# ComputationalPhysiology/oasisx

Measured on AMD Instinct MI355X. Metric: time-steps/sec, 3D Taylor-Green 128^3 P2-P1 (with pressure-CG SpMV GB/s in roofline), higher is better.
Workload: dtype f64

## Files before the change

include/oasisx_hip.h:

```cpp
#ifndef OASISX_HIP_H
#define OASISX_HIP_H

#include <stddef.h>
#include <stdint.h>

#ifdef __cplusplus
extern "C" {
#endif

#define OX_KV 2
#define OX_ROW_BLOCK_WAVES 8
#define OX_ROW_BLOCK_LDS (134 * 1024)
#define OX_SLICE 64

#define OX_CONVERGED_RTOL 2
#define OX_CONVERGED_ATOL 3
#define OX_CONVERGED_ITS 4
#define OX_DIVERGED_ITS (-3)
#define OX_DIVERGED_DTOL (-4)
#define OX_DIVERGED_BREAKDOWN (-5)
#define OX_DIVERGED_NANORINF (-9)

#define OX_KSP_CG 1
#define OX_KSP_BCGS 2
// ... 12 lines not shown
  const int32_t *cols;
  double *vals;
  const uint16_t *cols16;
  const int32_t *cbase;
  const uint8_t *vcode;
  const double *vdict;
  const int32_t *ib_slices;
  int32_t n_interior;
  int32_t n_wb_interior;
  const int64_t *ps_ptr;
  const uint32_t *ps_code;
  const int32_t *ps_base;
  const int32_t *wb_slices;
  const uint16_t *wb_waves;
  const int64_t *wb_ptr;
  const int32_t *wlist;
  const int64_t *wt_ptr;
  const uint16_t *wcode;
  const uint8_t *wvcode;
  int32_t n_wblocks;
  int32_t w_max;
  int32_t levels;
  int32_t w_cap;
} ox_sell;
#define OX_SPMV_LEVELS(mask) (32 | ((mask) & 31))

typedef struct {
  int32_t gdim;
  int32_t reserved;
  int64_t n_cells;
  const double *geom;
} ox_cells;

typedef struct {
  int32_t n_slices;
  int32_t nd;
  const int64_t *adj_ptr;
  const int32_t *adj_cell;
  const uint8_t *adj_loc;
} ox_adj;

typedef struct ox_dist ox_dist;
typedef struct ox_mg ox_mg;

typedef struct {
  int32_t reason[4];
  int32_t its[4];
  double rnorm[4];
// ... 90 lines not shown
int ox_value_dictionary(const double *vals, int64_t n_slots, int ncomp, void *codes, double *dict, int *n_dict,
                        void *stream);
int ox_pair_stream_size(const ox_sell *A, const int32_t *row_len, int64_t *ps_ptr, int64_t *n_codes, void *stream);
int ox_window_retile(const ox_sell *A, const int64_t *wt_ptr, const void *src, int elem_bytes, void *dst, void *stream);
int ox_pair_stream_fill(const ox_sell *A, const int32_t *row_len, int64_t *ps_ptr, uint32_t *ps_code,
                        int32_t *ps_base, int64_t *n_wide, void *stream);
int ox_gather_images(const double *src, int64_t n_src, const int32_t *image_dof, int64_t n_images, int ncomp, double *dst,
                     void *stream);
int ox_malloc(size_t bytes, void **out);
int ox_free(void *p);
int ox_memset(void *p, int value, size_t bytes, void *stream);
int ox_synchronize(void *stream);

int ox_version(void);
const char *ox_last_error(void);
int ox_sell_kv(void);
int ox_device_info(int *n_cu, char *name, int name_len);

int ox_spmv(const ox_sell *A, const double *x, double *y, int ncomp, const ox_dist *dist,
            void *stream);

int ox_sell_compress_cols(const ox_sell *A, uint16_t *cols16, int32_t *cbase, int64_t *n_compressed,
                          void *stream);

int ox_spmv_multi(int v2s, int gdim, const ox_sell *A, const double *x, const double *base, double scale,
                  double *y, const ox_dist *dist, void *stream);
int ox_assemble_rect(int family, int row_degree, int col_degree, const ox_cells *cells, const ox_adj *adj,
                     const uint8_t *adj_pos, int pw, const ox_sell *A, void *stream);

int ox_axpby(int64_t n, double a, const double *x, double b, const double *y, double *z,
             void *stream);
int ox_dot(int64_t n_rows, int ncomp, const double *x, const double *y, double *out_host,
           const ox_dist *dist, void *stream);

int ox_set_bc(double *b, const int32_t *dofs, const double *g, int64_t n, int ncomp, int comp,
              void *stream);

int ox_scatter_add(double *b, const int32_t *rows, const double *y, int64_t n, int ncomp, int comp,
                   double scale, void *stream);

int ox_zero_rows(const ox_sell *A, const int32_t *rows, int64_t n, double diag, void *stream);
int ox_zero_rows_au(const ox_sell *A, const int32_t *rows, int64_t n, double diag, double *au,
                    const double *u1, int ncomp, void *stream);
int ox_zero_rows_cols(const ox_sell *A, const uint8_t *is_bc, double diag, void *stream);

int ox_assemble_matrix(int kind, const ox_cells *cells, const ox_space_info *space, const ox_sell *A, int row_blocks,
// ... 228 lines not shown
```

oasisx_amd/_lib.py:

```python
from __future__ import annotations

import ctypes as C
import os

_HERE = os.path.dirname(os.path.abspath(__file__))
LIB_PATH = os.environ.get("OX_LIB_PATH") or os.path.join(_HERE, "liboasisx_hip.so")

KSP_CG, KSP_BCGS, KSP_CG_SINGLE, KSP_BCGS_MERGED, KSP_CG_MERGED = 1, 2, 3, 4, 5
KSP_CG_MG = 6
MG_MAX_DEGREE = 8
ROW_BLOCK_WAVES, ROW_BLOCK_LDS = 8, 134 * 1024
CONVERGED_RTOL, CONVERGED_ATOL, CONVERGED_ITS = 2, 3, 4
DIVERGED_ITS, DIVERGED_DTOL, DIVERGED_BREAKDOWN, DIVERGED_NANORINF = -3, -4, -5, -9


class OasisxHipError(RuntimeError):
    pass


class ox_sell(C.Structure):
    _fields_ = [
        ("n_rows", C.c_int64),
        ("n_cols", C.c_int64),
        ("n_slices", C.c_int32),
# ... 2 lines not shown
        ("cols", C.c_void_p),
        ("vals", C.c_void_p),
        ("cols16", C.c_void_p),
        ("cbase", C.c_void_p),
        ("vcode", C.c_void_p),
        ("vdict", C.c_void_p),
        ("ib_slices", C.c_void_p),
        ("n_interior", C.c_int32),
        ("n_wb_interior", C.c_int32),
        ("ps_ptr", C.c_void_p),
        ("ps_code", C.c_void_p),
        ("ps_base", C.c_void_p),
        ("wb_slices", C.c_void_p),
        ("wb_waves", C.c_void_p),
        ("wb_ptr", C.c_void_p),
        ("wlist", C.c_void_p),
        ("wt_ptr", C.c_void_p),
        ("wcode", C.c_void_p),
        ("wvcode", C.c_void_p),
        ("n_wblocks", C.c_int32),
        ("w_max", C.c_int32),
        ("levels", C.c_int32),
        ("w_cap", C.c_int32),
    ]


class ox_window_info(C.Structure):
    _fields_ = [
        ("n_wblocks", C.c_int32),
        ("w_max", C.c_int32),
        ("n_list", C.c_int64),
        ("n_tiles", C.c_int64),
        ("n_over_16bit", C.c_int64),
        ("wb_slices", C.c_void_p),
        ("wb_waves", C.c_void_p),
        ("wb_ptr", C.c_void_p),
        ("wlist", C.c_void_p),
        ("wt_ptr", C.c_void_p),
        ("wcode", C.c_void_p),
    ]


class ox_cells(C.Structure):
    _fields_ = [
        ("gdim", C.c_int32),
        ("reserved", C.c_int32),
# ... 207 lines not shown
    "ox_mesh_create_periodic": (_I, [_P, _L, _P, _P, _L, _L, _I, _I, _I, C.POINTER(_D), C.POINTER(_P)]),
    "ox_mesh_destroy": (_I, [_P]),
    "ox_space_create": (_I, [_P, _I, _I, C.POINTER(_P)]),
    "ox_space_create_ordered": (_I, [_P, _I, _I, _I, C.POINTER(_P)]),
    "ox_mesh_create_sub": (_I, [_P, _L, _P, _L, _I, _I, C.POINTER(_D), C.POINTER(_D), _I, _I, _L, C.POINTER(_P)]),
    "ox_space_create_part": (_I, [_P, _I, _I, _P, _L, _I, _L, C.POINTER(_P)]),
    "ox_space_view": (_I, [_P, C.POINTER(ox_space_info)]),
    "ox_space_windows": (_I, [_P, C.POINTER(ox_window_info)]),
    "ox_space_windows_split": (_I, [_P, _I, C.POINTER(ox_window_info)]),
    "ox_space_destroy": (_I, [_P]),
    "ox_rect_create": (_I, [_P, _P, C.POINTER(_P)]),
    "ox_rect_view": (_I, [_P, C.POINTER(ox_rect_info)]),
    "ox_rect_destroy": (_I, [_P]),
    "ox_value_dictionary": (_I, [_P, _L, _I, _P, _P, C.POINTER(_I), _P]),
    "ox_pair_stream_size": (_I, [C.POINTER(ox_sell), _P, _P, C.POINTER(_L), _P]),
    "ox_pair_stream_fill": (_I, [C.POINTER(ox_sell), _P, _P, _P, _P, C.POINTER(_L), _P]),
    "ox_gather_images": (_I, [_P, _L, _P, _L, _I, _P, _P]),
    "ox_malloc": (_I, [C.c_size_t, C.POINTER(_P)]),
    "ox_free": (_I, [_P]),
    "ox_memset": (_I, [_P, _I, C.c_size_t, _P]),
    "ox_synchronize": (_I, [_P]),
    "ox_spmv": (_I, [C.POINTER(ox_sell), _P, _P, _I, _P, _P]),
    "ox_sell_compress_cols": (_I, [C.POINTER(ox_sell), _P, _P, C.POINTER(_L), _P]),
    "ox_spmv_multi": (_I, [_I, _I, C.POINTER(ox_sell), _P, _P, _D, _P, _P, _P]),
    "ox_assemble_rect": (_I, [_I, _I, _I, C.POINTER(ox_cells), C.POINTER(ox_adj), _P, _I, C.POINTER(ox_sell), _P]),
    "ox_axpby": (_I, [_L, _D, _P, _D, _P, _P, _P]),
    "ox_dot": (_I, [_L, _I, _P, _P, C.POINTER(_D), _P, _P]),
    "ox_set_bc": (_I, [_P, _P, _P, _L, _I, _I, _P]),
    "ox_scatter_add": (_I, [_P, _P, _P, _L, _I, _I, _D, _P]),
    "ox_zero_rows": (_I, [C.POINTER(ox_sell), _P, _L, _D, _P]),
    "ox_zero_rows_au": (_I, [C.POINTER(ox_sell), _P, _L, _D, _P, _P, _I, _P]),
    "ox_zero_rows_cols": (_I, [C.POINTER(ox_sell), _P, _D, _P]),
    "ox_assemble_matrix": (_I, [_I, C.POINTER(ox_cells), C.POINTER(ox_space_info), C.POINTER(ox_sell), _I, _P]),
    "ox_assemble_weights": (_I, [_I, C.POINTER(ox_cells), C.POINTER(ox_adj), _L, _P, _P]),
    "ox_assemble_load_vector": (_I, [C.POINTER(ox_cells), C.POINTER(ox_adj), _L, _I, _I, _P, _P, _P, _P]),
    "ox_assemble_first": (_I, [C.POINTER(ox_cells), C.POINTER(ox_space_info), C.POINTER(ox_sell), C.POINTER(ox_sell),
                               C.POINTER(ox_sell), C.POINTER(ox_first_args), _I, _P]),
    "ox_eddy_viscosity": (_I, [_I, _I, C.POINTER(ox_cells), _P, _P, _D, _P, _P]),
    "ox_eddy_viscosity_damped": (_I, [_I, _I, C.POINTER(ox_cells), _P, _P, _D, C.POINTER(ox_vandriest), _P, _P]),
    "ox_viscosity_law": (_I, [_I, _I, C.POINTER(ox_cells), _P, _P, C.POINTER(_D), _I, _P, _P]),
    "ox_assemble_stress_transpose": (_I, [_I, C.POINTER(ox_cells), _P, C.POINTER(ox_adj), _L, _P, _P, _D, _P, _P]),
    "ox_flow_cells": (_I, [_I, C.POINTER(ox_cells), _P, _P, _P, _D, _D, _P, _P, _P, _P]),
    "ox_flow_reduce": (_I, [_L, _P, _P, _L, _L, _P]),
    "ox_stats_accumulate": (_I, [_I, _L, _P, _L, _D, _D, _P, _P, _P]),
    "ox_profile_cells": (_I, [_I, C.POINTER(ox_cells), _P, _I, _I, C.POINTER(_P), C.POINTER(_L), _P, _P, _L, _P, _P, _P]),
    "ox_profile_update": (_I, [_I, _L, _P, _P, _P, _D, _D, _I, _P, _P, _P, _P, _P]),
# ... 117 lines not shown
```

oasisx_amd/csrc/ox_ksp.hip:

```cpp
#include "ox_kernels.h"
#include "ox_ksp_dev.h"
#include "ox_p2p.h"
#include <type_traits>

struct KspPart2 {
  const double *partial;
  int nparts, nv;
};

__device__ __forceinline__ void ksp_gather2(const double *__restrict__ partial, int nparts, int nv, const KspPart2 &B,
                                            double (&v)[OX_MAX_NV]) {
  ox_gather_partials(partial, nparts, nv, v);
  if (B.nv > 0) {
    double w[OX_MAX_NV];
    ox_gather_partials(B.partial, B.nparts, B.nv, w);
#pragma unroll
    for (int i = 0; i < OX_MAX_NV; ++i)
#pragma unroll
      for (int j = 0; j < OX_MAX_NV; ++j)
        if (j == i - nv && j < B.nv) v[i] = w[j];
  }
}


// ... 1569 lines not shown
  } else {
    V.r = vec[0], V.rhat = vec[1], V.p = vec[2], V.v = vec[3], V.s = vec[4], V.t = vec[5];
    if (guess && !ax0) {
      if (ox_spmv_dist(A, x, V.t, NC, OX_EPI_NONE, nullptr, nullptr, nullptr, nullptr, dist, st)) return -1;
    }
    hipLaunchKernelGGL((k_bcgs_init<NC>), dim3(C.nb), dim3(256), 0, st, n, b, x, (guess && ax0) ? ax0 : V.t, C.dinv, V.r,
                       V.rhat, V.p, V.v, guess, C.partial);
    OX_LAUNCH_CHECK();
    KSP_SYNC(PH_BCGS_INIT, C.partial, C.nb, 2 * NC);
  }
  bool first = true;
  int it = 0;
  bool tail_done = false;
  for (;;) {
    tail_done = false;
    if (ksp_iterate<NC>(C, V, P, check_every, ahead && NC == 1, it, first, H)) return -1;
    int live = -1;
    if (NC > 1 && !hs->done) live = ksp_last_live(hs, NC);
    if (live >= 0) {
      double *const *cv = C.narrow;
      KspVecs W{};
      double *src[8] = {V.x, V.r, V.z, V.p, V.q, V.rhat, V.v, nullptr};
      double **dst[8] = {&W.x, &W.r, &W.z, &W.p, &W.q, &W.rhat, &W.v, nullptr};
      if (cg) src[2] = nullptr;
      if (cgs) {
        src[2] = V.u, dst[2] = &W.u;
        src[4] = V.s, dst[4] = &W.s;
        src[5] = V.w, dst[5] = &W.w;
        src[6] = nullptr;
      }
      for (int i = 0; i < 7; ++i) {
        *dst[i] = cv[i];
        if (!src[i]) continue;
        hipLaunchKernelGGL(k_extract_col, dim3(C.nb), dim3(256), 0, st, n, src[i], NC, live, cv[i]);
        OX_LAUNCH_CHECK();
      }
      if (!cgs) {
        W.s = cv[2];
        W.t = cv[4];
      }
      KspParams P1 = P;
      P1.nc = 1;
      P1.c0 = live;
      it += check_every;
      if (ksp_iterate<1>(C, W, P1, check_every, ahead, it, first, H)) return -1;
      if (cg) {
        hipLaunchKernelGGL((k_cg_update2<1>), dim3(C.nb), dim3(256), 0, st, n, C.S, P1.c0, W.x, W.r, C.D, W.p, 1);
// ... 93 lines not shown
```

oasisx_amd/csrc/ox_spmv.hip:

```cpp
#include "ox_common.h"
#include "ox_kernels.h"
#include <stdlib.h>
#include <type_traits>

thread_local char ox_err_buf[512] = "";

extern "C" int ox_version(void) { return 101; }
extern "C" const char *ox_last_error(void) { return ox_err_buf; }
extern "C" int ox_sell_kv(void) { return OX_KV; }

extern "C" int ox_device_info(int *n_cu, char *name, int name_len) {
  int dev = 0;
  OX_HIP(hipGetDevice(&dev));
  hipDeviceProp_t p;
  OX_HIP(hipGetDeviceProperties(&p, dev));
  if (n_cu) *n_cu = p.multiProcessorCount;
  if (name && name_len > 0) {
    strncpy(name, p.gcnArchName, name_len - 1);
    name[name_len - 1] = 0;
  }
  return 0;
}

template <int NC, int EPI, int VAR>
// ... 44 lines not shown
      if (VAR & 4) {
        const unsigned cc = __builtin_nontemporal_load(vcp + (size_t)k * 64);
        v.x = dict[cc & 0xff];
        v.y = dict[cc >> 8];
      } else if (VAR & 1) {
        const v2d vv = __builtin_nontemporal_load(reinterpret_cast<const v2d *>(vp + (size_t)k * 64));
        v.x = vv.x;
        v.y = vv.y;
      } else {
        v = vp[(size_t)k * 64];
      }
      return v;
    };
    auto mac = [&](double2 v, int c0, int c1) {
      const double *x0 = x + (size_t)c0 * NC;
      const double *x1 = x + (size_t)c1 * NC;
#pragma unroll
      for (int cc = 0; cc < NC; ++cc) acc[cc] = fma(v.x, x0[cc], acc[cc]);
#pragma unroll
      for (int cc = 0; cc < NC; ++cc) acc[cc] = fma(v.y, x1[cc], acc[cc]);
    };
    const int2 *__restrict__ cb =
        (VAR & 2) ? reinterpret_cast<const int2 *>(A.cbase) + (base >> 7) : nullptr;
    if ((VAR & 2) && cb[0].x >= 0) {
      const v2h *__restrict__ hp = reinterpret_cast<const v2h *>(A.cols16 + base) + lane;
#pragma unroll 4
      for (int k = 0; k < npair; ++k) {
        const double2 v = load_vals(k);
        const v2h d = __builtin_nontemporal_load(hp + (size_t)k * 64);
        const int2 b = cb[k];
        const int dx = d.x, dy = d.y;
        mac(v, ((dx & 0x8000) ? b.y : b.x) + (dx & 0x7fff), ((dy & 0x8000) ? b.y : b.x) + (dy & 0x7fff));
      }
    } else {
      const int2 *__restrict__ cp = reinterpret_cast<const int2 *>(A.cols + base) + lane;
#pragma unroll 4
      for (int k = 0; k < npair; ++k) {
        const double2 v = load_vals(k);
        int2 c;
        if (VAR & 1) {
          const v2i ci = __builtin_nontemporal_load(reinterpret_cast<const v2i *>(cp + (size_t)k * 64));
          c.x = ci.x;
          c.y = ci.y;
        } else {
          c = cp[(size_t)k * 64];
        }
        mac(v, c.x, c.y);
// ... 393 lines not shown
    if (threadIdx.x == 0) {
#pragma unroll
      for (int i = 0; i < NV; ++i) partial[(size_t)blockIdx.x * NV + i] = s[i];
    }
  }
}

#include <mutex>
static const int *ox_zero_flag(hipStream_t st) {
  static std::mutex mu;
  static int *z[16] = {};
  int dev = 0;
  if (hipGetDevice(&dev) != hipSuccess || dev < 0 || dev >= 16) return nullptr;
  std::lock_guard<std::mutex> lock(mu);
  if (!z[dev]) {
    int *p = nullptr;
    if (hipMalloc(&p, 64) != hipSuccess) return nullptr;
    if (hipMemsetAsync(p, 0, 64, st) != hipSuccess || hipStreamSynchronize(st) != hipSuccess) return nullptr;
    z[dev] = p;
  }
  return z[dev];
}

#define OX_SPMV_DEFAULT_VARIANT 31
static inline int spmv_levels(const ox_sell *A) { return (A->levels & 32) ? (A->levels & 31) : OX_SPMV_DEFAULT_VARIANT; }

static int spmv_window_cap(const ox_sell *A, int ncomp, const int32_t *list) {
  if (list && !(A->ib_slices && (list == A->ib_slices || list == A->ib_slices + A->n_interior))) return 0;
  if (!(spmv_levels(A) & 16) || !A->wcode || !A->wt_ptr || !A->wlist || !A->wb_ptr || !A->wb_slices ||
      !A->wb_waves || A->n_wblocks <= 0 || ncomp < 1 || ncomp > 3)
    return 0;
  const int dflt = ncomp == 1 ? 6144 : (ncomp == 2 ? 3072 : 2176);
  const int cap = A->w_cap > 0 ? A->w_cap : dflt;
  return A->w_max < cap ? A->w_max : cap;
}
static inline int spmv_window_grid_n(int nblocks) { return (nblocks + 7) & ~7; }
static inline void spmv_window_range(const ox_sell *A, const int32_t *list, int n_list, int *first, int *count) {
  if (!list) *first = 0, *count = A->n_wblocks;
  else if (list == A->ib_slices && n_list == A->n_interior) *first = 0, *count = A->n_wb_interior;
  else *first = A->n_wb_interior, *count = A->n_wblocks - A->n_wb_interior;
}

static thread_local OxEpiDinv g_epi_dinv{nullptr, nullptr};
void ox_spmv_set_epilogue_dinv(const uint8_t *code, const double *dict) { g_epi_dinv = OxEpiDinv{code, dict}; }

static int spmv_launch_list(const ox_sell *A, const double *x, double *y, int ncomp, int epi,
                            const double *dinv, const double *aux, double *partial, const int *done,
                            hipStream_t st, const int32_t *list, int n_list) {
  const int nblk = list ? ox_spmv_blocks_n(n_list) : ox_spmv_blocks(A);
  if (nblk == 0) return 0;
  const int lv = spmv_levels(A);
  int var = (A->cols16 && A->cbase) ? (lv & 7) : (lv & 1);
  const bool pairs = (lv & 8) && A->ps_ptr && A->ps_code && A->ps_base;
  if ((var & 6) != 6 || !A->vcode || !A->vdict || A->n_dict < 1 || A->n_dict > 256) var &= 3;
  else var = 7;
  const int w_cap = pairs ? 0 : spmv_window_cap(A, ncomp, list);
  if (w_cap > 0) {
    const bool codes = var == 7 && A->wvcode;
    int wb0 = 0, wbn = 0;
    spmv_window_range(A, list, n_list, &wb0, &wbn);
    if (wbn == 0) return 0;
    const int wgrid = spmv_window_grid_n(wbn);
    const size_t lds = (size_t)w_cap * ncomp * sizeof(double);
#define OX_WIN_CASE(NC, E)                                                                                          \
  if (ncomp == NC && epi == E) {                                                                                    \
    auto go = [&](auto kern) -> int {                                                                               \
      if (lds > 48 * 1024)                                                                                          \
        OX_HIP(hipFuncSetAttribute(reinterpret_cast<const void *>(kern), hipFuncAttributeMaxDynamicSharedMemorySize, \
                                   (int)lds));                                                                      \
      if (ox_prof_on) ox_prof_start(OX_TAG_SPMV(NC, E), st, A->n_rows);                                             \
      hipLaunchKernelGGL(kern, dim3(wgrid), dim3(256), lds, st, *A, x, y, dinv, aux, partial, done, w_cap, g_epi_dinv, wb0, wbn); \
      if (ox_prof_on) ox_prof_stop(st);                                                                             \
      OX_LAUNCH_CHECK();                                                                                            \
      return 0;                                                                                                     \
    };                                                                                                              \
    return codes ? go(k_spmv_win<NC, E, 5>) : go(k_spmv_win<NC, E, 1>);                                             \
  }
#define OX_WIN_NC(NC)                                                                                   \
  OX_WIN_CASE(NC, OX_EPI_NONE) OX_WIN_CASE(NC, OX_EPI_DOT) OX_WIN_CASE(NC, OX_EPI_BCGS_V) OX_WIN_CASE(NC, OX_EPI_BCGS_T) \
  OX_WIN_CASE(NC, OX_EPI_BCGS_T5) OX_WIN_CASE(NC, OX_EPI_CG_M2)
    OX_WIN_NC(1) OX_WIN_NC(2) OX_WIN_NC(3)
#undef OX_WIN_NC
#undef OX_WIN_CASE
  }
#define OX_SPMV_LAUNCH(NC, E, V)                                                                   \
  hipLaunchKernelGGL((k_spmv<NC, E, V>), dim3(nblk), dim3(256), 0, st, *A, x, y, dinv, aux, partial, done, list, n_list, g_epi_dinv)
#define OX_SPMV_CASE(NC, E)                                                                     \
  if (ncomp == NC && epi == E) {                                                                \
    if (ox_prof_on) ox_prof_start(OX_TAG_SPMV(NC, E), st, A->n_rows);                                      \
    if (var == 7 && pairs) {                                                                    \
      const int *dz = done ? done : ox_zero_flag(st);                                             \
      if (!dz) OX_FAIL("ox_spmv: no device flag");                                              \
      hipLaunchKernelGGL((k_spmv_ps<NC, E>), dim3(nblk), dim3(256), 0, st, *A, x, y, dinv, aux, partial, dz, list, n_list, g_epi_dinv); \
    } else if (var == 7) OX_SPMV_LAUNCH(NC, E, 7);                                              \
    else if (var == 3) OX_SPMV_LAUNCH(NC, E, 3);                                                \
    else if (var == 2) OX_SPMV_LAUNCH(NC, E, 2);                                                \
    else if (var == 1) OX_SPMV_LAUNCH(NC, E, 1);                                                \
    else OX_SPMV_LAUNCH(NC, E, 0);                                                              \
    if (ox_prof_on) ox_prof_stop(st);                                                           \
    OX_LAUNCH_CHECK();                                                                          \
    return 0;                                                                                   \
  }
#define OX_SPMV_NC(NC)               \
  OX_SPMV_CASE(NC, OX_EPI_NONE)      \
  OX_SPMV_CASE(NC, OX_EPI_DOT)       \
  OX_SPMV_CASE(NC, OX_EPI_BCGS_V)    \
  OX_SPMV_CASE(NC, OX_EPI_BCGS_T)    \
  OX_SPMV_CASE(NC, OX_EPI_BCGS_T5)   \
  OX_SPMV_CASE(NC, OX_EPI_CG_M2)
  OX_SPMV_NC(1) OX_SPMV_NC(2) OX_SPMV_NC(3)
#undef OX_SPMV_NC
#undef OX_SPMV_CASE
  OX_FAIL("ox_spmv: unsupported ncomp=%d epi=%d", ncomp, epi);
}

int ox_spmv_launch(const ox_sell *A, const double *x, double *y, int ncomp, int epi,
                   const double *dinv, const double *aux, double *partial, const int *done,
                   hipStream_t st) {
  return spmv_launch_list(A, x, y, ncomp, epi, dinv, aux, partial, done, st, nullptr, 0);
}

static bool ox_overlap_on(const ox_sell *A, const ox_dist *dist) {
  if (!(dist && dist->n_peers > 0 && A->ib_slices && A->n_interior > 0)) return false;
  if (dist->overlap >= 0) return dist->overlap != 0;
  return !(dist->comm && !dist->p2p && !dist->halo_cb);
}

static int spmv_parts_of(const ox_sell *A, int ncomp, const int32_t *list, int n_list) {
  const bool pairs = (spmv_levels(A) & 8) && A->ps_ptr && A->ps_code && A->ps_base;
  if (!pairs && spmv_window_cap(A, ncomp, list) > 0) {
    int wb0 = 0, wbn = 0;
    spmv_window_range(A, list, n_list, &wb0, &wbn);
    return wbn == 0 ? 0 : spmv_window_grid_n(wbn);
  }
  return list ? ox_spmv_blocks_n(n_list) : ox_spmv_blocks(A);
// ... 76 lines not shown
extern "C" int ox_sell_compress_cols(const ox_sell *A, uint16_t *cols16, int32_t *cbase,
                                     int64_t *n_compressed, void *stream) {
  if (!A || !cols16 || !cbase) OX_FAIL("ox_sell_compress_cols: null argument");
  hipStream_t st = ox_stream(stream);
  if (n_compressed) *n_compressed = 0;
  if (A->n_slices == 0) return 0;
  unsigned long long *cnt = nullptr;
  if (n_compressed) {
    OX_HIP(hipMalloc(&cnt, sizeof(*cnt)));
    OX_HIP(hipMemsetAsync(cnt, 0, sizeof(*cnt), st));
  }
  hipLaunchKernelGGL(k_compress_cols, dim3((A->n_slices + 3) / 4), dim3(256), 0, st, *A, cols16, cbase, cnt);
  OX_LAUNCH_CHECK();
  if (n_compressed) {
    unsigned long long h = 0;
    OX_HIP(hipMemcpyAsync(&h, cnt, sizeof(h), hipMemcpyDeviceToHost, st));
    OX_HIP(hipStreamSynchronize(st));
    OX_HIP(hipFree(cnt));
    *n_compressed = (int64_t)h;
  }
  return 0;
}

template <int GD, int V2S, bool DICT>
__global__ __launch_bounds__(256) void k_spmv_multi(ox_sell A, const double *__restrict__ x,
                                                    const double *__restrict__ base, double scale,
                                                    double *__restrict__ y) {
  __shared__ double dict[DICT ? 256 : 1];
  if constexpr (DICT) {
    if ((int)threadIdx.x < A.n_dict) dict[threadIdx.x] = A.vdict[threadIdx.x];
    __syncthreads();
  }
  const int ngroups = (A.n_slices + 3) >> 2;
  const int chunk = (ngroups + 7) >> 3;
  const int g = (blockIdx.x & 7) * chunk + (blockIdx.x >> 3);
  if ((int)(blockIdx.x >> 3) >= chunk || g >= ngroups) return;
  const int slice = __builtin_amdgcn_readfirstlane(g * 4 + (threadIdx.x >> 6)), lane = threadIdx.x & 63;
  if (slice >= A.n_slices) return;
  const int64_t row = (int64_t)slice * 64 + lane;
  const int64_t sbase = A.slice_ptr[slice];
  const int npair = (int)((A.slice_ptr[slice + 1] - sbase) >> 7);
  const int2 *__restrict__ cp = reinterpret_cast<const int2 *>(A.cols + sbase) + lane;
  double acc[GD];
#pragma unroll
  for (int d = 0; d < GD; ++d) acc[d] = 0.0;
  auto mac = [&](const double (&v)[2 * GD], int c0, int c1) {
// ... 513 lines not shown
```

oasisx_amd/fem.py:

```python
from __future__ import annotations

import ctypes as C
import itertools

import numpy as np
import torch

from . import _lib
from .mesh import Mesh

KV = 2
SLICE = 64
default_scalar_type = np.float64


def local_edges(gdim: int):
    return [(1, 2), (0, 2), (0, 1)] if gdim == 2 else [(2, 3), (1, 3), (1, 2), (0, 3), (0, 2), (0, 1)]


import os as _os


def default_tile_bits(mesh: Mesh) -> int:
    env = _os.environ.get("OX_TILE_BITS")
# ... 144 lines not shown
    for k in per.axes:
        cut[k] = float(per.hi[k] - per.atol[k])
    keep = (X < cut).all(dim=2)
    x = torch.full((n, d), float("nan"), dtype=torch.float64, device=dev)
    x[cd0[keep]] = X[keep]
    return x


class SellPattern:

    def __init__(self, n_rows, n_cols, slice_ptr, cols, row_len, widths, nnz=None, row_blk=None):
        self.n_rows, self.n_cols = int(n_rows), int(n_cols)
        self.slice_ptr = slice_ptr
        self.cols = cols
        self.row_len = row_len
        self.widths = widths
        self.n_slices = int(widths.shape[0])
        self.size = int(cols.shape[0])
        self.nnz = int(row_len.sum().item()) if nnz is None else int(nnz)
        self.device = cols.device
        self.dist = None
        self.cols16 = self.cbase = None
        self.frac16 = 0.0
        self.ib_slices, self.n_interior = None, 0
        w = torch.from_numpy(widths.astype(np.int64))
        order = torch.argsort(w, stable=True)
        ws = w[order]
        uw, counts = torch.unique_consecutive(ws, return_counts=True)
        self.bin_width, self.bin_ptr = merge_small_bins(uw.numpy().astype(np.int32),
                                                        np.concatenate([[0], np.cumsum(counts.numpy())]).astype(np.int64))
        self.bin_slices = order.to(torch.int32).to(self.device)
        if row_blk is None:
            bp, big = row_blocks(widths)
            row_blk = (torch.from_numpy(bp).to(self.device), big)
        self.row_blk_ptr, self.row_blk_entries = row_blk
        self.n_row_blocks = int(self.row_blk_ptr.shape[0]) - 1

    def split_interior(self, n_owned: int):
        if self.n_slices == 0 or self.size == 0:
            return
        width = torch.from_numpy(self.widths.astype(np.int64)).to(self.device) * SLICE
        sl = torch.repeat_interleave(torch.arange(self.n_slices, device=self.device), width)
        ghost = torch.zeros(self.n_slices, dtype=torch.int32, device=self.device)
        ghost.index_put_((sl,), (self.cols >= n_owned).to(torch.int32), accumulate=True)
        interior = torch.nonzero(ghost == 0).reshape(-1)
        boundary = torch.nonzero(ghost > 0).reshape(-1)
# ... 94 lines not shown
            bs = torch.repeat_interleave(blk_of_slice[s0:s1], slot_per_slice[s0:s1])
            code = torch.searchsorted(ukey, bs * ncols + self.cols[a:b].to(torch.int64)) - wb_ptr[bs]
            code = torch.where(big[bs], torch.zeros_like(code), code)
            wcode[a:b] = (code & 0xffff).to(torch.int32).to(torch.int16)
        npair = width // KV
        wt_ptr = torch.zeros(ns + 1, dtype=torch.int64, device=dev)
        wt_ptr[1:] = torch.cumsum((npair + 1) // 2, 0)
        n_tiles = int(wt_ptr[-1].item())
        plain = _lib.ox_sell(self.n_rows, self.n_cols, self.n_slices, 0, self.slice_ptr.data_ptr(), self.cols.data_ptr())
        tiled = torch.empty(n_tiles * 256, dtype=torch.int16, device=dev)
        _lib.check(_lib.load().ox_window_retile(C.byref(plain), _lib.ptr(wt_ptr), _lib.ptr(wcode), 2, _lib.ptr(tiled),
                                                _lib.current_stream()), "ox_window_retile")
        del wcode
        self.wb_slices, self.wb_waves = wb_slices.contiguous(), sched.to(torch.int32).to(torch.int16).contiguous()
        self.wb_ptr, self.wlist, self.wcode, self.wt_ptr = wb_ptr, wlist.contiguous(), tiled, wt_ptr
        self.n_wblocks, self.w_max = nb, w_max
        wq = torch.quantile(w_all.to(torch.float64), torch.tensor([0.5, 0.9, 0.99], dtype=torch.float64, device=dev))
        self.w_stats = {"blocks": nb, "w_mean": float(w_all.to(torch.float64).mean().item()), "w_max": w_max,
                        "w_p50_p90_p99": [int(v) for v in wq.tolist()],
                        "share_over_2176": float((w_all > 2176).to(torch.float64).mean().item()),
                        "list_bytes": int(wlist.numel()) * 4, "over_16bit": int(big.sum().item())}
        return True

    def struct(self, vals: torch.Tensor, compress: bool = True) -> _lib.ox_sell:
        assert vals.shape[0] % self.size == 0 and vals.dtype == torch.float64
        c16 = cb = None
        if compress and self.device.type == "cuda" and self.size > 0:
            if self.cols16 is None:
                self.cols16 = torch.empty(self.size, dtype=torch.int16, device=self.device)
                self.cbase = torch.empty(2 * (self.size // (SLICE * KV)), dtype=torch.int32, device=self.device)
                plain = _lib.ox_sell(self.n_rows, self.n_cols, self.n_slices, 0, self.slice_ptr.data_ptr(),
                                     self.cols.data_ptr(), None, None, None, None, None)
                n16 = C.c_int64(0)
                _lib.check(_lib.load().ox_sell_compress_cols(C.byref(plain), _lib.ptr(self.cols16),
                                                             _lib.ptr(self.cbase), C.byref(n16),
                                                             _lib.current_stream()), "ox_sell_compress_cols")
                self.frac16 = n16.value / self.size
            c16, cb = self.cols16.data_ptr(), self.cbase.data_ptr()
        S = _lib.ox_sell(self.n_rows, self.n_cols, self.n_slices, 0, self.slice_ptr.data_ptr(),
                         self.cols.data_ptr(), vals.data_ptr(), c16, cb, None, None)
        if self.ib_slices is not None:
            S.ib_slices, S.n_interior = self.ib_slices.data_ptr(), self.n_interior
        if getattr(self, "wcode", None) is not None:
            S.wb_slices, S.wb_waves, S.wb_ptr = self.wb_slices.data_ptr(), self.wb_waves.data_ptr(), self.wb_ptr.data_ptr()
            S.wlist, S.wcode, S.n_wblocks, S.w_max = self.wlist.data_ptr(), self.wcode.data_ptr(), self.n_wblocks, self.w_max
            S.wt_ptr = self.wt_ptr.data_ptr()
            S.n_wb_interior = int(getattr(self, "n_wb_interior", None) or 0)
        return S

    def slot_rows_k(self):
        sp = self.slice_ptr.cpu().numpy()
        o = np.arange(self.size, dtype=np.int64)
        s = np.searchsorted(sp, o, side="right") - 1
        loc = o - sp[s]
        k = (loc // (SLICE * KV)) * KV + loc % KV
        lane = (loc % (SLICE * KV)) // KV
        return s * SLICE + lane, k

    def to_csr(self, vals: torch.Tensor):
        import scipy.sparse as sp

        rows, k = self.slot_rows_k()
        rl = np.zeros(self.n_slices * SLICE, dtype=np.int64)
# ... 1175 lines not shown
```

oasisx_amd/la.py:

```python
from __future__ import annotations

import ctypes as C
import os

import torch

from . import _lib
from .fem import SellPattern


def _env_int(name):
    try:
        return int(os.environ[name])
    except (KeyError, ValueError):
        return None


ENV_SPMV_LEVELS = _env_int("OX_SPMV_VARIANT")
ENV_WIN_CAP = _env_int("OX_WIN_CAP")


def _apply_schedule(struct, levels, w_cap):
    struct.levels = 0 if levels is None else (32 | (int(levels) & 31))
    struct.w_cap = 0 if not w_cap else int(w_cap)


class SellMatrix:

    def __init__(self, pattern: SellPattern, symmetric: bool = False, name: str = "A"):
        self.pattern = pattern
        self.vals = pattern.new_values()
        self.symmetric = symmetric
        self.name = name
        self.version = 0
        self.vcode = self.vdict = self._vc_version = None
        self.ps_ptr = self.ps_code = self.ps_base = None
        self.ps_wide = 0
        self.wvcode = None
        self._struct = pattern.struct(self.vals)
        self.levels, self.w_cap = ENV_SPMV_LEVELS, ENV_WIN_CAP
        _apply_schedule(self._struct, self.levels, self.w_cap)

    def set_levels(self, mask: int | None, w_cap: int | None = None):
        self.levels = mask
        if w_cap is not None:
            self.w_cap = w_cap or None
        _apply_schedule(self._struct, self.levels, self.w_cap)

    @property
    def struct(self) -> _lib.ox_sell:
        return self._struct

    def ref(self):
        if self._vc_version is not None and self._vc_version != self.version:
            self._drop_codes()
        return C.byref(self._struct)

    def _drop_codes(self):
        self.vcode = self.vdict = self._vc_version = None
        self._struct.vcode = self._struct.vdict = None
        self._struct.n_dict = 0
        self.ps_ptr = self.ps_code = self.ps_base = None
        self._struct.ps_ptr = self._struct.ps_code = self._struct.ps_base = None
        self.wvcode = None
        self._struct.wvcode = None

    def freeze(self, block: int = 1 << 27, pairs: str = "auto") -> bool:
        P = self.pattern
        if P.device.type != "cuda" or P.cols16 is None or P.size == 0:
            return False
        code = torch.empty(P.size, dtype=torch.uint8, device=P.device)
        vdict = torch.zeros(256, dtype=torch.float64, device=P.device)
        nd = C.c_int(0)
        _lib.check(_lib.load().ox_value_dictionary(_lib.ptr(self.vals), P.size, 1, _lib.ptr(code), _lib.ptr(vdict),
                                                   C.byref(nd), _lib.current_stream()), "ox_value_dictionary")
        if nd.value == 0:
            return False
        self.vcode, self.vdict = code, vdict[: nd.value]
        self._vc_version = self.version
        self._struct.vcode, self._struct.vdict = self.vcode.data_ptr(), self.vdict.data_ptr()
        self._struct.n_dict = int(nd.value)
        if pairs != "never":
            self._build_pair_stream(force=pairs == "always")
        if getattr(P, "wt_ptr", None) is not None and self.ps_code is None:
            self.wvcode = torch.empty(int(P.wt_ptr[-1].item()) * 256, dtype=torch.uint8, device=P.device)
            _lib.check(_lib.load().ox_window_retile(C.byref(self._struct), _lib.ptr(P.wt_ptr), _lib.ptr(self.vcode), 1,
                                                    _lib.ptr(self.wvcode), _lib.current_stream()), "ox_window_retile")
            self._struct.wvcode = self.wvcode.data_ptr()
        return True

    def _build_pair_stream(self, force: bool = False):
        P, lib = self.pattern, _lib.load()
        ps_ptr = torch.empty(P.n_slices + 1, dtype=torch.int64, device=P.device)
        n = C.c_int64(0)
        _lib.check(lib.ox_pair_stream_size(C.byref(self._struct), _lib.ptr(P.row_len), _lib.ptr(ps_ptr), C.byref(n),
                                           _lib.current_stream()), "ox_pair_stream_size")
        if n.value == 0 or (not force and n.value > 0.72 * P.size):
            return
        code = torch.empty(n.value, dtype=torch.int32, device=P.device)
        base = torch.empty(2 * (n.value // 256), dtype=torch.int32, device=P.device)
        wide = C.c_int64(0)
        _lib.check(lib.ox_pair_stream_fill(C.byref(self._struct), _lib.ptr(P.row_len), _lib.ptr(ps_ptr), _lib.ptr(code),
                                           _lib.ptr(base), C.byref(wide), _lib.current_stream()), "ox_pair_stream_fill")
        self.ps_ptr, self.ps_code, self.ps_base, self.ps_wide = ps_ptr, code, base, int(wide.value)
        self._struct.ps_ptr, self._struct.ps_code, self._struct.ps_base = ps_ptr.data_ptr(), code.data_ptr(), base.data_ptr()

    def getSize(self):
        return (self.pattern.n_rows, self.pattern.n_cols)

    def to_scipy(self):
        return self.pattern.to_csr(self.vals)

# ... 70 lines not shown
```

Baseline: 12.29.

## Encode SELL column and value codes as per-wavefront contiguous runs in SpMV

Adds a run-length encoding of SELL slice columns: each 64-lane column vector is described by up to four contiguous pieces (header with break lanes plus base columns). A matching per-run value-code word is built for dictionary-compressed matrices. The SpMV kernel gains variants that rebuild column indices and values from these small headers instead of streaming the 16-bit column array and the per-entry value codes, which cuts index traffic in the bandwidth-bound CG SpMV. Runs are enabled by default when at least half the positions can be encoded. Positions that cannot be encoded fall back to the coded path, at the cost of extra branching and header loads. It also drops the q vector from a CG workspace copy list.

```diff
diff --git a/include/oasisx_hip.h b/include/oasisx_hip.h
--- a/include/oasisx_hip.h
+++ b/include/oasisx_hip.h
@@ -58,8 +58,11 @@
   int32_t w_max;
   int32_t levels;
   int32_t w_cap;
+  const uint32_t *crun_hdr;
+  const int32_t *crun_base;
+  const uint32_t *vrun;
 } ox_sell;
-#define OX_SPMV_LEVELS(mask) (32 | ((mask) & 31))
+#define OX_SPMV_LEVELS(mask) (32 | ((mask) & 31) | (((mask) & 32) << 1))
 
 typedef struct {
   int32_t gdim;
@@ -196,6 +199,10 @@
 
 int ox_sell_compress_cols(const ox_sell *A, uint16_t *cols16, int32_t *cbase, int64_t *n_compressed,
                           void *stream);
+
+int ox_sell_build_col_runs(const ox_sell *A, uint32_t *crun_hdr, int32_t *crun_base, int64_t *n_on_runs,
+                           void *stream);
+int ox_sell_build_val_runs(const ox_sell *A, uint32_t *vrun, int64_t *n_on_runs, void *stream);
 
 int ox_spmv_multi(int v2s, int gdim, const ox_sell *A, const double *x, const double *base, double scale,
                   double *y, const ox_dist *dist, void *stream);
diff --git a/oasisx_amd/_lib.py b/oasisx_amd/_lib.py
--- a/oasisx_amd/_lib.py
+++ b/oasisx_amd/_lib.py
@@ -48,6 +48,9 @@
         ("w_max", C.c_int32),
         ("levels", C.c_int32),
         ("w_cap", C.c_int32),
+        ("crun_hdr", C.c_void_p),
+        ("crun_base", C.c_void_p),
+        ("vrun", C.c_void_p),
     ]
 
 
@@ -301,6 +304,8 @@
     "ox_synchronize": (_I, [_P]),
     "ox_spmv": (_I, [C.POINTER(ox_sell), _P, _P, _I, _P, _P]),
     "ox_sell_compress_cols": (_I, [C.POINTER(ox_sell), _P, _P, C.POINTER(_L), _P]),
+    "ox_sell_build_col_runs": (_I, [C.POINTER(ox_sell), _P, _P, C.POINTER(_L), _P]),
+    "ox_sell_build_val_runs": (_I, [C.POINTER(ox_sell), _P, C.POINTER(_L), _P]),
     "ox_spmv_multi": (_I, [_I, _I, C.POINTER(ox_sell), _P, _P, _D, _P, _P, _P]),
     "ox_assemble_rect": (_I, [_I, _I, _I, C.POINTER(ox_cells), C.POINTER(ox_adj), _P, _I, C.POINTER(ox_sell), _P]),
     "ox_axpby": (_I, [_L, _D, _P, _D, _P, _P, _P]),
diff --git a/oasisx_amd/csrc/ox_ksp.hip b/oasisx_amd/csrc/ox_ksp.hip
--- a/oasisx_amd/csrc/ox_ksp.hip
+++ b/oasisx_amd/csrc/ox_ksp.hip
@@ -1615,7 +1615,7 @@
       KspVecs W{};
       double *src[8] = {V.x, V.r, V.z, V.p, V.q, V.rhat, V.v, nullptr};
       double **dst[8] = {&W.x, &W.r, &W.z, &W.p, &W.q, &W.rhat, &W.v, nullptr};
-      if (cg) src[2] = nullptr;
+      if (cg) src[2] = src[4] = nullptr;
       if (cgs) {
         src[2] = V.u, dst[2] = &W.u;
         src[4] = V.s, dst[4] = &W.s;
diff --git a/oasisx_amd/csrc/ox_spmv.hip b/oasisx_amd/csrc/ox_spmv.hip
--- a/oasisx_amd/csrc/ox_spmv.hip
+++ b/oasisx_amd/csrc/ox_spmv.hip
@@ -90,7 +90,103 @@
     };
     const int2 *__restrict__ cb =
         (VAR & 2) ? reinterpret_cast<const int2 *>(A.cbase) + (base >> 7) : nullptr;
-    if ((VAR & 2) && cb[0].x >= 0) {
+    if ((VAR & 8) && cb[0].x >= 0) {
+      const v2h *__restrict__ hp = reinterpret_cast<const v2h *>(A.cols16 + base) + lane;
+      const uint2 *__restrict__ hq = reinterpret_cast<const uint2 *>(A.crun_hdr) + (base >> 7);
+      const int4 *__restrict__ bq = reinterpret_cast<const int4 *>(A.crun_base) + (base >> 6);
+      const uint2 *__restrict__ wq = (VAR & 4) ? reinterpret_cast<const uint2 *>(A.vrun) + (base >> 7) : nullptr;
+      auto coded_pair = [&](int k) {
+        const double2 v = load_vals(k);
+        const v2h d = __builtin_nontemporal_load(hp + (size_t)k * 64);
+        const int2 b = cb[k];
+        const int dx = d.x, dy = d.y;
+        mac(v, ((dx & 0x8000) ? b.y : b.x) + (dx & 0x7fff), ((dy & 0x8000) ? b.y : b.x) + (dy & 0x7fff));
+      };
+      auto group = [&](auto ng_tag, int k, const uint2 *h, const uint2 *w) {
+        constexpr int NG = decltype(ng_tag)::value;
+        bool coded = false, pieces = false;
+#pragma unroll
+        for (int i = 0; i < NG; ++i) {
+          const unsigned n0 = h[i].x & 0xffu, n1 = h[i].y & 0xffu;
+          coded = coded || n0 == 0 || n1 == 0;
+          pieces = pieces || n0 > 1 || n1 > 1;
+          if (VAR & 4) coded = coded || w[i].x == 0xffffffffu || w[i].y == 0xffffffffu;
+        }
+        if (coded) {
+#pragma unroll
+          for (int i = 0; i < NG; ++i) coded_pair(k + i);
+        } else if (!pieces) {
+          double2 v[NG];
+          int c0[NG], c1[NG];
+#pragma unroll
+          for (int i = 0; i < NG; ++i) {
+            if (VAR & 4) v[i].x = dict[w[i].x & 0xffu], v[i].y = dict[w[i].y & 0xffu];
+            else v[i] = load_vals(k + i);
+            c0[i] = bq[2 * (k + i)].x + lane;
+            c1[i] = bq[2 * (k + i) + 1].x + lane;
+          }
+#pragma unroll
+          for (int i = 0; i < NG; ++i) mac(v[i], c0[i], c1[i]);
+        } else {
+          double2 v[NG];
+          int c0[NG], c1[NG];
+          auto decode = [&](unsigned hh, int4 B, unsigned ww, int &col, double &val) {
+            const int b1 = (int)((hh >> 8) & 0xffu), b2 = (int)((hh >> 16) & 0xffu), b3 = (int)(hh >> 24);
+            const bool p1 = lane >= b1, p2 = lane >= b2, p3 = lane >= b3;
+            int bs = B.x;
+            bs = p1 ? B.y : bs;
+            bs = p2 ? B.z : bs;
+            bs = p3 ? B.w : bs;
+            col = bs + lane;
+            if (VAR & 4) {
+              unsigned cd = ww & 0xffu;
+              cd = p1 ? ((ww >> 8) & 0xffu) : cd;
+              cd = p2 ? ((ww >> 16) & 0xffu) : cd;
+              cd = p3 ? (ww >> 24) : cd;
+              val = dict[cd];
+            }
+          };
+#pragma unroll
+          for (int i = 0; i < NG; ++i) {
+            if (!(VAR & 4)) v[i] = load_vals(k + i);
+            decode(h[i].x, bq[2 * (k + i)], (VAR & 4) ? w[i].x : 0u, c0[i], v[i].x);
+            decode(h[i].y, bq[2 * (k + i) + 1], (VAR & 4) ? w[i].y : 0u, c1[i], v[i].y);
+          }
+#pragma unroll
+          for (int i = 0; i < NG; ++i) mac(v[i], c0[i], c1[i]);
+        }
+      };
+      int k = 0;
+      if (npair >= 4) {
+        uint2 h[4], w[4];
+#pragma unroll
+        for (int i = 0; i < 4; ++i) {
+          h[i] = hq[i];
+          if (VAR & 4) w[i] = wq[i];
+        }
+        for (; k + 4 <= npair; k += 4) {
+          const int kn = min(k + 4, npair - 4);
+          uint2 hn[4], wn[4];
+#pragma unroll
+          for (int i = 0; i < 4; ++i) {
+            hn[i] = hq[kn + i];
+            if (VAR & 4) wn[i] = wq[kn + i];
+          }
+          group(std::integral_constant<int, 4>{}, k, h, w);
+#pragma unroll
+          for (int i = 0; i < 4; ++i) {
+            h[i] = hn[i];
+            if (VAR & 4) w[i] = wn[i];
+          }
+        }
+      }
+      for (; k < npair; ++k) {
+        const uint2 h1 = hq[k];
+        uint2 w1 = make_uint2(0u, 0u);
+        if (VAR & 4) w1 = wq[k];
+        group(std::integral_constant<int, 1>{}, k, &h1, &w1);
+      }
+    } else if ((VAR & 2) && cb[0].x >= 0) {
       const v2h *__restrict__ hp = reinterpret_cast<const v2h *>(A.cols16 + base) + lane;
 #pragma unroll 4
       for (int k = 0; k < npair; ++k) {
@@ -530,8 +626,9 @@
   return z[dev];
 }
 
-#define OX_SPMV_DEFAULT_VARIANT 31
-static inline int spmv_levels(const ox_sell *A) { return (A->levels & 32) ? (A->levels & 31) : OX_SPMV_DEFAULT_VARIANT; }
+#define OX_SPMV_RUNS 64
+#define OX_SPMV_DEFAULT_VARIANT (31 | OX_SPMV_RUNS)
+static inline int spmv_levels(const ox_sell *A) { return (A->levels & 32) ? (A->levels & (31 | OX_SPMV_RUNS)) : OX_SPMV_DEFAULT_VARIANT; }
 
 static int spmv_window_cap(const ox_sell *A, int ncomp, const int32_t *list) {
   if (list && !(A->ib_slices && (list == A->ib_slices || list == A->ib_slices + A->n_interior))) return 0;
@@ -562,6 +659,9 @@
   const bool pairs = (lv & 8) && A->ps_ptr && A->ps_code && A->ps_base;
   if ((var & 6) != 6 || !A->vcode || !A->vdict || A->n_dict < 1 || A->n_dict > 256) var &= 3;
   else var = 7;
+  const bool runs = (lv & OX_SPMV_RUNS) && A->crun_hdr && A->crun_base &&
+                    ((var == 3 && (ncomp == 1 || (ncomp == 3 && (epi == OX_EPI_NONE || epi == OX_EPI_BCGS_V)))) ||
+                     (var == 7 && A->vrun && ncomp == 3));
   const int w_cap = pairs ? 0 : spmv_window_cap(A, ncomp, list);
   if (w_cap > 0) {
     const bool codes = var == 7 && A->wvcode;
@@ -593,6 +693,7 @@
   }
 #define OX_SPMV_LAUNCH(NC, E, V)                                                                   \
   hipLaunchKernelGGL((k_spmv<NC, E, V>), dim3(nblk), dim3(256), 0, st, *A, x, y, dinv, aux, partial, done, list, n_list, g_epi_dinv)
+#define OX_RUNS_F64(NC, E) (NC == 1 || (NC == 3 && (E == OX_EPI_NONE || E == OX_EPI_BCGS_V)))
 #define OX_SPMV_CASE(NC, E)                                                                     \
   if (ncomp == NC && epi == E) {                                                                \
     if (ox_prof_on) ox_prof_start(OX_TAG_SPMV(NC, E), st, A->n_rows);                                      \
@@ -600,7 +701,9 @@
       const int *dz = done ? done : ox_zero_flag(st);                                             \
       if (!dz) OX_FAIL("ox_spmv: no device flag");                                              \
       hipLaunchKernelGGL((k_spmv_ps<NC, E>), dim3(nblk), dim3(256), 0, st, *A, x, y, dinv, aux, partial, dz, list, n_list, g_epi_dinv); \
-    } else if (var == 7) OX_SPMV_LAUNCH(NC, E, 7);                                              \
+    } else if (var == 7 && runs && NC == 3) OX_SPMV_LAUNCH(NC, E, (NC == 3 ? 15 : 7));          \
+    else if (var == 3 && runs && OX_RUNS_F64(NC, E)) OX_SPMV_LAUNCH(NC, E, (OX_RUNS_F64(NC, E) ? 11 : 3)); \
+    else if (var == 7) OX_SPMV_LAUNCH(NC, E, 7);                                                \
     else if (var == 3) OX_SPMV_LAUNCH(NC, E, 3);                                                \
     else if (var == 2) OX_SPMV_LAUNCH(NC, E, 2);                                                \
     else if (var == 1) OX_SPMV_LAUNCH(NC, E, 1);                                                \
@@ -619,6 +722,7 @@
   OX_SPMV_NC(1) OX_SPMV_NC(2) OX_SPMV_NC(3)
 #undef OX_SPMV_NC
 #undef OX_SPMV_CASE
+#undef OX_RUNS_F64
   OX_FAIL("ox_spmv: unsupported ncomp=%d epi=%d", ncomp, epi);
 }
 
@@ -741,6 +845,124 @@
   return 0;
 }
 
+__device__ __forceinline__ int ox_run_piece_base(int lane, unsigned hdr, int b0, int b1v, int b2v, int b3v) {
+  const int l1 = (int)((hdr >> 8) & 0xffu), l2 = (int)((hdr >> 16) & 0xffu), l3 = (int)(hdr >> 24);
+  int bs = b0;
+  bs = lane >= l1 ? b1v : bs;
+  bs = lane >= l2 ? b2v : bs;
+  bs = lane >= l3 ? b3v : bs;
+  return bs;
+}
+
+__global__ __launch_bounds__(256) void k_build_col_runs(ox_sell A, uint32_t *__restrict__ hdr, int32_t *__restrict__ rbase,
+                                                        unsigned long long *n_ok) {
+  const int slice = blockIdx.x * 4 + (threadIdx.x >> 6), lane = threadIdx.x & 63;
+  if (slice >= A.n_slices) return;
+  const int64_t base = A.slice_ptr[slice];
+  const int npair = (int)((A.slice_ptr[slice + 1] - base) >> 7);
+  const int2 *cp = reinterpret_cast<const int2 *>(A.cols + base) + lane;
+  unsigned long long covered = 0;
+  for (int k = 0; k < npair; ++k) {
+    const int2 c2 = cp[(size_t)k * 64];
+    for (int j = 0; j < 2; ++j) {
+      const int c = j ? c2.y : c2.x;
+      const int left = __shfl_up(c, 1, 64);
+      const unsigned long long brk = __ballot(lane > 0 && c != left + 1);
+      const int nb = __popcll(brk);
+      int l[3] = {64, 64, 64};
+      unsigned long long m = brk;
+      for (int i = 0; i < 3 && m; ++i) {
+        l[i] = __ffsll((long long)m) - 1;
+        m &= m - 1;
+      }
+      const int mine = c - lane;
+      const int b0 = __shfl(mine, 0, 64), b1 = __shfl(mine, l[0] & 63, 64), b2 = __shfl(mine, l[1] & 63, 64),
+                b3 = __shfl(mine, l[2] & 63, 64);
+      unsigned h = (unsigned)(nb + 1) | ((unsigned)l[0] << 8) | ((unsigned)l[1] << 16) | ((unsigned)l[2] << 24);
+      const int dec = ox_run_piece_base(lane, h, b0, l[0] < 64 ? b1 : 0, l[1] < 64 ? b2 : 0, l[2] < 64 ? b3 : 0) + lane;
+      const bool ok = nb <= 3 && __all(dec == c);
+      if (!ok) h = (h & ~0xffu);
+      const int64_t pos = (base >> 6) + 2 * k + j;
+      if (lane == 0) hdr[pos] = h;
+      if (lane < 4) {
+        const int bv = lane == 0 ? b0 : (lane == 1 ? b1 : (lane == 2 ? b2 : b3));
+        rbase[pos * 4 + lane] = (lane == 0 || l[lane > 0 ? lane - 1 : 0] < 64) ? bv : 0;
+      }
+      covered += ok ? 1 : 0;
+    }
+  }
+  if (lane == 0 && n_ok && covered) atomicAdd(n_ok, covered);
+}
+
+__global__ __launch_bounds__(256) void k_build_val_runs(ox_sell A, uint32_t *__restrict__ vrun, unsigned long long *n_ok) {
+  const int slice = blockIdx.x * 4 + (threadIdx.x >> 6), lane = threadIdx.x & 63;
+  if (slice >= A.n_slices) return;
+  const int64_t base = A.slice_ptr[slice];
+  const int npair = (int)((A.slice_ptr[slice + 1] - base) >> 7);
+  const uint8_t *vc = A.vcode + base + 2 * lane;
+  unsigned long long covered = 0;
+  for (int k = 0; k < npair; ++k) {
+    for (int j = 0; j < 2; ++j) {
+      const int64_t pos = (base >> 6) + 2 * k + j;
+      const unsigned h = A.crun_hdr[pos];
+      const int code = vc[(size_t)k * 128 + j];
+      const int l1 = (int)((h >> 8) & 0xffu), l2 = (int)((h >> 16) & 0xffu), l3 = (int)(h >> 24);
+      const int c0 = __shfl(code, 0, 64), c1 = __shfl(code, l1 & 63, 64), c2 = __shfl(code, l2 & 63, 64),
+                c3 = __shfl(code, l3 & 63, 64);
+      const int dec = ox_run_piece_base(lane, h, c0, c1, c2, c3);
+      const bool ok = (h & 0xffu) != 0 && __all(dec == code);
+      if (lane == 0)
+        vrun[pos] = ok ? ((unsigned)c0 | (l1 < 64 ? (unsigned)c1 << 8 : 0u) | (l2 < 64 ? (unsigned)c2 << 16 : 0u) |
+                          (l3 < 64 ? (unsigned)c3 << 24 : 0u))
+                       : 0xffffffffu;
+      covered += ok ? 1 : 0;
+    }
+  }
+  if (lane == 0 && n_ok && covered) atomicAdd(n_ok, covered);
+}
+
+static int ox_run_count(unsigned long long *cnt, int64_t *out, hipStream_t st) {
+  unsigned long long h = 0;
+  OX_HIP(hipMemcpyAsync(&h, cnt, sizeof(h), hipMemcpyDeviceToHost, st));
+  OX_HIP(hipStreamSynchronize(st));
+  OX_HIP(hipFree(cnt));
+  *out = (int64_t)h;
+  return 0;
+}
+
+extern "C" int ox_sell_build_col_runs(const ox_sell *A, uint32_t *crun_hdr, int32_t *crun_base, int64_t *n_on_runs,
+                                      void *stream) {
+  if (!A || !crun_hdr || !crun_base) OX_FAIL("ox_sell_build_col_runs: null argument");
+  hipStream_t st = ox_stream(stream);
+  if (n_on_runs) *n_on_runs = 0;
+  if (A->n_slices == 0) return 0;
+  unsigned long long *cnt = nullptr;
+  if (n_on_runs) {
+    OX_HIP(hipMalloc(&cnt, sizeof(*cnt)));
+    OX_HIP(hipMemsetAsync(cnt, 0, sizeof(*cnt), st));
+  }
+  hipLaunchKernelGGL(k_build_col_runs, dim3((A->n_slices + 3) / 4), dim3(256), 0, st, *A, crun_hdr, crun_base, cnt);
+  OX_LAUNCH_CHECK();
+  return n_on_runs ? ox_run_count(cnt, n_on_runs, st) : 0;
+}
+
+extern "C" int ox_sell_build_val_runs(const ox_sell *A, uint32_t *vrun, int64_t *n_on_runs, void *stream) {
+  if (!A || !vrun) OX_FAIL("ox_sell_build_val_runs: null argument");
+  if (!A->crun_hdr || !A->vcode) OX_FAIL("ox_sell_build_val_runs: the matrix carries no column runs or no value codes");
+  if (A->n_dict < 1 || A->n_dict > 255) OX_FAIL("ox_sell_build_val_runs: n_dict=%d, 1..255 needed", A->n_dict);
+  hipStream_t st = ox_stream(stream);
+  if (n_on_runs) *n_on_runs = 0;
+  if (A->n_slices == 0) return 0;
+  unsigned long long *cnt = nullptr;
+  if (n_on_runs) {
+    OX_HIP(hipMalloc(&cnt, sizeof(*cnt)));
+    OX_HIP(hipMemsetAsync(cnt, 0, sizeof(*cnt), st));
+  }
+  hipLaunchKernelGGL(k_build_val_runs, dim3((A->n_slices + 3) / 4), dim3(256), 0, st, *A, vrun, cnt);
+  OX_LAUNCH_CHECK();
+  return n_on_runs ? ox_run_count(cnt, n_on_runs, st) : 0;
+}
+
 template <int GD, int V2S, bool DICT>
 __global__ __launch_bounds__(256) void k_spmv_multi(ox_sell A, const double *__restrict__ x,
                                                     const double *__restrict__ base, double scale,
diff --git a/oasisx_amd/fem.py b/oasisx_amd/fem.py
--- a/oasisx_amd/fem.py
+++ b/oasisx_amd/fem.py
@@ -190,6 +190,8 @@
         self.dist = None
         self.cols16 = self.cbase = None
         self.frac16 = 0.0
+        self.crun_hdr = self.crun_base = None
+        self.frac_runs = None
         self.ib_slices, self.n_interior = None, 0
         w = torch.from_numpy(widths.astype(np.int64))
         order = torch.argsort(w, stable=True)
@@ -330,6 +332,25 @@
                         "list_bytes": int(wlist.numel()) * 4, "over_16bit": int(big.sum().item())}
         return True
 
+    RUNS_MIN_SHARE = 0.5
+
+    def build_col_runs(self, force: bool = False) -> bool:
+        if self.device.type != "cuda" or self.size == 0 or self.cols16 is None:
+            return False
+        if self.frac_runs is None or (force and self.crun_hdr is None):
+            npos = self.size // SLICE
+            hdr = torch.empty(npos, dtype=torch.int32, device=self.device)
+            base = torch.empty(4 * npos, dtype=torch.int32, device=self.device)
+            plain = _lib.ox_sell(self.n_rows, self.n_cols, self.n_slices, 0, self.slice_ptr.data_ptr(),
+                                 self.cols.data_ptr())
+            n = C.c_int64(0)
+            _lib.check(_lib.load().ox_sell_build_col_runs(C.byref(plain), _lib.ptr(hdr), _lib.ptr(base), C.byref(n),
+                                                          _lib.current_stream()), "ox_sell_build_col_runs")
+            self.frac_runs = n.value / npos
+            if force or self.frac_runs >= self.RUNS_MIN_SHARE:
+                self.crun_hdr, self.crun_base = hdr, base
+        return self.crun_hdr is not None
+
     def struct(self, vals: torch.Tensor, compress: bool = True) -> _lib.ox_sell:
         assert vals.shape[0] % self.size == 0 and vals.dtype == torch.float64
         c16 = cb = None
@@ -347,6 +368,8 @@
             c16, cb = self.cols16.data_ptr(), self.cbase.data_ptr()
         S = _lib.ox_sell(self.n_rows, self.n_cols, self.n_slices, 0, self.slice_ptr.data_ptr(),
                          self.cols.data_ptr(), vals.data_ptr(), c16, cb, None, None)
+        if c16 is not None and self.build_col_runs():
+            S.crun_hdr, S.crun_base = self.crun_hdr.data_ptr(), self.crun_base.data_ptr()
         if self.ib_slices is not None:
             S.ib_slices, S.n_interior = self.ib_slices.data_ptr(), self.n_interior
         if getattr(self, "wcode", None) is not None:
diff --git a/oasisx_amd/la.py b/oasisx_amd/la.py
--- a/oasisx_amd/la.py
+++ b/oasisx_amd/la.py
@@ -21,7 +21,7 @@
 
 
 def _apply_schedule(struct, levels, w_cap):
-    struct.levels = 0 if levels is None else (32 | (int(levels) & 31))
+    struct.levels = 0 if levels is None else (32 | (int(levels) & 31) | ((int(levels) & 32) << 1))
     struct.w_cap = 0 if not w_cap else int(w_cap)
 
 
@@ -37,6 +37,8 @@
         self.ps_ptr = self.ps_code = self.ps_base = None
         self.ps_wide = 0
         self.wvcode = None
+        self.vrun = None
+        self.frac_vruns = None
         self._struct = pattern.struct(self.vals)
         self.levels, self.w_cap = ENV_SPMV_LEVELS, ENV_WIN_CAP
         _apply_schedule(self._struct, self.levels, self.w_cap)
@@ -64,6 +66,8 @@
         self._struct.ps_ptr = self._struct.ps_code = self._struct.ps_base = None
         self.wvcode = None
         self._struct.wvcode = None
+        self.vrun = self.frac_vruns = None
+        self._struct.vrun = None
 
     def freeze(self, block: int = 1 << 27, pairs: str = "auto") -> bool:
         P = self.pattern
@@ -87,7 +91,22 @@
             _lib.check(_lib.load().ox_window_retile(C.byref(self._struct), _lib.ptr(P.wt_ptr), _lib.ptr(self.vcode), 1,
                                                     _lib.ptr(self.wvcode), _lib.current_stream()), "ox_window_retile")
             self._struct.wvcode = self.wvcode.data_ptr()
+        self._build_val_runs()
         return True
+
+    def _build_val_runs(self, force: bool = False):
+        P = self.pattern
+        if P.crun_hdr is None or self.vcode is None or not 1 <= self._struct.n_dict <= 255:
+            return
+        self._struct.crun_hdr, self._struct.crun_base = P.crun_hdr.data_ptr(), P.crun_base.data_ptr()
+        vrun = torch.empty(P.size // 64, dtype=torch.int32, device=P.device)
+        n = C.c_int64(0)
+        _lib.check(_lib.load().ox_sell_build_val_runs(C.byref(self._struct), _lib.ptr(vrun), C.byref(n),
+                                                      _lib.current_stream()), "ox_sell_build_val_runs")
+        self.frac_vruns = n.value / vrun.numel()
+        if force or self.frac_vruns >= P.RUNS_MIN_SHARE:
+            self.vrun = vrun
+            self._struct.vrun = vrun.data_ptr()
 
     def _build_pair_stream(self, force: bool = False):
         P, lib = self.pattern, _lib.load()
```

Result: no change. 12.43 (median of 4 runs) (+1.1%).
